# TheCacophonyProject/classifier-pipeline

Hardware: AMD Instinct MI355X
Metric: CPTV frames/s end-to-end (track+classify) at 160x120 (higher is better)
Workload: dtype u16/i32 track stage (f32 normalise, f64 gates); f32 crop/tile; f32 CNN (stride-1 3x3 convs of stages 2-4 (+ the stride-2 one): two fp16 planes per operand rounded to nearest (11 + 11 significand bits), power-of-two range scaling, 3 fp16 MFMAs per K step, device-side rerun in the exact split if an ac

## Files before the change

### classifier-pipeline_amd/csrc/cpx_api.cpp

```cpp
#include <hip/hip_runtime.h>

#include <algorithm>
#include <cmath>
#include <cstdio>
#include <cstdlib>
#include <cstring>
#include <new>
#include <string>
#include <vector>

#include "cpx_internal.h"
#include "cpx_schedule_core.h"

static_assert(sizeof(cpx_component) == 32, "cpx_component layout is part of the ABI");
static_assert(sizeof(cpx_frame_info) == 80, "cpx_frame_info layout is part of the ABI");
static_assert(sizeof(cpx_frame_meta) == 24, "cpx_frame_meta layout is part of the ABI");
static_assert(sizeof(cpx_config) == 48, "cpx_config layout is part of the ABI");
static_assert(sizeof(cpx_region_ref) == 24 && sizeof(cpx_track_limits) == 32 && sizeof(cpx_crop_req) == 32,
              "classification request layouts are part of the ABI");
static_assert(sizeof(cpx_filter_params) == 72 && sizeof(cpx_track_summary) == 120,
              "end-of-clip layouts are part of the ABI");
static_assert(sizeof(cpx_region) == 56, "cpx_region layout is part of the ABI");
static_assert(sizeof(cpx_track_record) == 32, "cpx_track_record layout is part of the ABI");
static_assert(sizeof(cpx_track_params) == 120, "cpx_track_params layout is part of the ABI");
// ... 79 lines not shown
    return CPX_ERR_HIP;
  }
  h->wtab_len = 65536;
  h->wtab_host.resize(h->wtab_len);
  std::vector<double>& wt = h->wtab_host;
  double w = 0.0;
  for (int k = 0; k < h->wtab_len; ++k) {
    wt[k] = w;
    w = w + cfg->weight_add;
  }
  if (cfg->denoise) {
    if (!cpx::nlm_supported(W, H)) {
      cpx_destroy(h);
      return CPX_ERR_UNSUPPORTED;
    }
    const int fixed_point_mult = (int)(2147483647LL / (21 * 21 * 255));
    std::vector<int> lut(64, 0);
    for (int a2 = 0; a2 < 64; ++a2) {
      const double wv = std::exp(-((double)a2 * (64.0 / 49.0)) / 9.0);
      const double wr = std::nearbyint((double)fixed_point_mult * wv);
      lut[a2] = (wr < 0.001 * fixed_point_mult) ? 0 : (int)wr;
    }
    if (lut[63] != 0 || h->nlm_lut_dev.grow(h, 64 * sizeof(int), "NLM weight table allocation") ||
        hipMemcpy(h->nlm_lut_dev.p, lut.data(), 64 * sizeof(int), hipMemcpyHostToDevice) != hipSuccess) {
      cpx_destroy(h);
      return CPX_ERR_HIP;
    }
  }
  std::vector<uint32_t> thr(h->wtab_len);
  for (int k = 0; k < h->wtab_len; ++k) {
    const double wk = wt[k], m = std::nearbyint(wk);
    const bool exact = (wk == m), near = !exact && std::fabs(wk - m) < 1e-6;
    double hi = near ? m + 1.0 : std::floor(wk) + 1.0;
    if (!(hi >= 0.0)) hi = 0.0;
    if (hi > 536870912.0) hi = 536870912.0;
    thr[k] = 2u * (uint32_t)hi - (near ? 1u : 0u);
  }
  if (h->wthr_dev.grow(h, thr.size() * sizeof(uint32_t), "threshold table allocation") ||
      hipMemcpy(h->wthr_dev.p, thr.data(), thr.size() * sizeof(uint32_t), hipMemcpyHostToDevice) != hipSuccess) {
    cpx_destroy(h);
    return CPX_ERR_HIP;
  }
  if (h->wtab_dev.grow(h, wt.size() * sizeof(double), "weight table allocation") ||
      hipMemcpy(h->wtab_dev.p, wt.data(), wt.size() * sizeof(double), hipMemcpyHostToDevice) != hipSuccess ||
      cpx::frame_kernel_attr_setup() != 0) {
    cpx_destroy(h);
    return CPX_ERR_HIP;
  }
  if (const char* env = std::getenv("CPX_TRACK_PACKED_STATE")) h->packed_state_ok = std::atoi(env) != 0;
  if (const char* env = std::getenv("CPX_CNN_FUSE_CONV1")) h->fuse_conv1 = std::atoi(env) != 0;
  if (const char* env = std::getenv("CPX_TRACK_PER_STEP")) h->track_per_step = std::atoi(env) != 0;
  if (const char* env = std::getenv("CPX_CNN_FUSE_SHORTCUT")) h->fuse_shortcut = std::atoi(env) != 0;
  if (const char* env = std::getenv("CPX_CNN_SHORTCUT_FP16")) h->shortcut_fp16 = std::atoi(env) != 0;
  if (const char* env = std::getenv("CPX_CNN_BLOCK_FUSION")) h->block_fusion = std::min(std::max(std::atoi(env), 0), 2);
  if (const char* env = std::getenv("CPX_CNN_MATH")) {
    if (!std::strcmp(env, "f32")) h->cnn_math = CPX_CNN_MATH_F32;
    else if (!std::strcmp(env, "bf16x3")) h->cnn_math = CPX_CNN_MATH_BF16X3;
    else if (!std::strcmp(env, "bf16x2")) h->cnn_math = CPX_CNN_MATH_BF16X2;
    else if (!std::strcmp(env, "fp16x2")) h->cnn_math = CPX_CNN_MATH_FP16X2;
  }
  *out = h;
  return CPX_OK;
}

static void release_buffers(cpx_handle* h, bool all) {
  for (DeviceBuffer* b : {&h->ws, &h->ws_assoc, &h->bf3_scratch, &h->cnn_arena, &h->graph_arena, &h->ir_scratch}) b->release();
  if (!all) return;
  for (DeviceBuffer* b : {&h->sched, &h->wtab_dev, &h->wthr_dev, &h->nlm_lut_dev, &h->cnn_ovf, &h->ir_bitmap}) b->release();
}

void cpx_destroy(cpx_handle* h) {
  if (!h) return;
  hipSetDevice(h->device);
  if (h->stream) hipStreamSynchronize(h->stream);
  for (cpx_cnn* c : h->cnns) cnn_free(c);
  h->cnns.clear();
  for (cpx_mog2* m : h->mog2s) mog2_free(m);
  h->mog2s.clear();
  for (cpx_graph* g : h->graphs) graph_free(g);
  h->graphs.clear();
  release_buffers(h, true);
  for (auto& e : h->conv_events) {
    hipEventDestroy(e.e0);
    hipEventDestroy(e.e1);
  }
  if (h->stream2) {
    hipStreamSynchronize(h->stream2);
    hipStreamDestroy(h->stream2);
  }
  if (h->ev_median) hipEventDestroy(h->ev_median);
  if (h->ev0) hipEventDestroy(h->ev0);
  if (h->ev1) hipEventDestroy(h->ev1);
  if (h->stream) hipStreamDestroy(h->stream);
  delete h;
}

const char* cpx_last_error(const cpx_handle* h) { return h ? h->err.c_str() : "null handle"; }

void* cpx_stream(cpx_handle* h) { return h ? (void*)h->stream : nullptr; }

static int join_medians(cpx_handle* h) {
  if (h->medians_pending) {
    h->medians_pending = false;
    CPX_HIP(h, hipStreamWaitEvent(h->stream, h->ev_median, 0));
  }
  return CPX_OK;
// ... 711 lines not shown
```

### classifier-pipeline_amd/csrc/cpx_api_cnn.cpp

```cpp
#include <hip/hip_runtime.h>

#include <algorithm>
#include <cmath>
#include <cstdio>
#include <cstdlib>
#include <new>
#include <utility>
#include <vector>

#include "cpx_internal.h"

static_assert(sizeof(cpx_wrresnet_block) == 56 && sizeof(cpx_wrresnet_params) == 1560,
              "cpx_wrresnet_params layout is part of the ABI");

struct cpx_cnn {
  cpx_handle* h = nullptr;
  cpx_wrresnet_params p{};
  std::vector<std::pair<const float*, void*>> split;
  float act_scale[3][CPX_WRRESNET_MAX_BLOCKS][2];
  float res_bound[3] = {0.0f, 0.0f, 0.0f};
  float sc_xscale[3] = {0.0f, 0.0f, 0.0f};
  void* sc_img[3] = {nullptr, nullptr, nullptr};
  double sc_wmax[3] = {-1.0, -1.0, -1.0};
  cpx_cnn() {
// ... 102 lines not shown
  Float32,
  Split,
  Fp16Pair,
  RerunOnly,
};

static int conv_run(cpx_handle* h, const cpx_conv_desc* d, const void* split_weights, const conv_fuse* fuse = nullptr,
                    const conv_half* hf = nullptr) {
  if (!h) return CPX_ERR_INVALID;
  if (!d || !d->in_dev || !d->out_dev || !d->weights_dev) return fail(h, CPX_ERR_INVALID, "cpx_conv2d: null argument");
  if (d->N < 1 || d->H < 1 || d->W < 1 || d->groups < 1 || d->Cin % d->groups || d->Cout % d->groups ||
      d->ksize < 1 || d->stride < 1 || (d->in_scale_dev == nullptr) != (d->in_shift_dev == nullptr))
    return fail(h, CPX_ERR_INVALID, "cpx_conv2d: bad descriptor");
  CPX_ENTER(h);
  if (!d->pad_same && (d->H < d->ksize || d->W < d->ksize)) return fail(h, CPX_ERR_INVALID, "cpx_conv2d: input smaller than kernel");
  cpx::ConvArgs a = conv_describe(*d, fuse);
  const bool split = split_math(h) && cpx::conv_bf3_supported(a);
  if (fuse && (!split || a.out_scale || a.residual))
    return fail(h, CPX_ERR_INVALID, "conv_run: shortcut fusion needs the split-operand kernel, no output scale, no residual");
  if (split) a.planes = h->cnn_math == CPX_CNN_MATH_BF16X2 ? 2 : 3;
  const conv_half bare;
  const conv_half& k = hf ? *hf : bare;
  const bool fp16 = split && h->cnn_math == CPX_CNN_MATH_FP16X2;
  const bool aliased = a.out == a.residual || a.out == a.in;
  const bool half = fp16 && cpx::conv_bf3_two_planes(a) && !aliased;
  const bool planes_out = fp16 && k.out_planes;
  const ConvRoute route = k.rerun_only ? ConvRoute::RerunOnly
                          : !split ? ConvRoute::Float32
                          : (half || planes_out) ? ConvRoute::Fp16Pair
                                                 : ConvRoute::Split;
  ConvTimer timer(h, h->conv_timing && route != ConvRoute::RerunOnly);
  if (!timer.ok()) return fail(h, CPX_ERR_HIP, "cpx_conv2d: event creation failed");
  int* word = nullptr;
  if (route == ConvRoute::Fp16Pair || route == ConvRoute::RerunOnly) {
    if (int rc = ensure_ovf_word(h)) return rc;
    if (!k.keep_flag) CPX_HIP(h, hipMemsetAsync(h->cnn_ovf.p, 0, sizeof(int), h->stream));
    word = h->cnn_ovf.as<int>() + k.word;
  }
  if (split && !split_weights) {
    if (int rc = h->bf3_scratch.grow(h, cpx::conv_bf3_weight_bytes(a), "cpx_conv2d: weight scratch allocation failed"))
      return rc;
    cpx::launch_split_weights(a, h->bf3_scratch.p, h->stream);
    split_weights = h->bf3_scratch.p;
  }
  int rc = 0;
  if (route == ConvRoute::Fp16Pair) {
    cpx::ConvArgs first = a;
    if (half) {
      first.planes = 2;
      first.half = 1;
      first.act_scale = k.act_scale;
      first.act_unscale = 1.0f / first.act_scale;
      first.in_planes = k.in_planes;
    }
    first.ovf = word;
    if (planes_out) {
      first.out_planes = 1;
      first.out_act_scale = k.out_act_scale;
    }
    rc = cpx::launch_conv_bf3(first, split_weights, h->stream);
  }
  a.guard = word;
  if (split) {
    if (rc == 0) rc = cpx::launch_conv_bf3(a, split_weights, h->stream);
    if (rc == -3) {
      if (fuse) return fail(h, CPX_ERR_UNSUPPORTED, "conv_run: batch too large for the fused-shortcut kernel (split the call)");
      rc = cpx::launch_conv(a, h->stream);
    }
  } else {
    rc = cpx::launch_conv(a, h->stream);
  }
  if (int trc = timer.commit((a.Cin / a.groups) * 10000 + (a.Cout / a.groups) * 10 + a.stride + (a.ksize == 1 ? 5 : 0),
                             2.0 * a.N * a.Ho * a.Wo * a.Cout * (double)(a.Cin / a.groups) * a.ksize * a.ksize))
    return trc;
  if (rc == -2) return fail(h, CPX_ERR_UNSUPPORTED, "cpx_conv2d: no kernel for this (channels per group, stride, kernel size)");
  if (rc != 0) return fail(h, CPX_ERR_HIP, "cpx_conv2d: kernel configuration failed");
  CPX_HIP(h, hipGetLastError());
  return CPX_OK;
}

static bool conv_can_fuse(const cpx_handle* h, int f, int groups) {
  return split_math(h) && cpx::conv_bf3_supported(conv_shape(0, 0, 0, f, f, groups, 3, 1, 1));
}

enum class BlockForm {
  OneLaunch,
  PlanesPair,
  Separate,
};
enum class Shortcut {
  Identity,
  FusedIntoSecond,
  OwnLaunch,
};
enum class Conv1 {
  NotHere,
  InFront,
  InsideBlock,
};
enum class Fusion { None, Block, BlockAndConv1 };

struct BlockPlan {
  int k, st, d;
  int stride, H, W, Ho, Wo, c_in, f;
  int word;
  BlockForm form;
// ... 537 lines not shown
```

### classifier-pipeline_amd/csrc/cpx_cnn_bf3.hip

```cpp
#include <hip/hip_runtime.h>

#include <algorithm>
#include <cstdlib>
#include <type_traits>

#include "cpx_cnn_dev.h"
#include "cpx_conv_layout_core.h"
#include "cpx_kernels.h"

namespace cpx {

namespace {

#define BF3_ENTRY_GUARD(H_)                          \
  if (H_) {                                          \
    if (*a.ovf != 0) return;                         \
  } else if (a.guard != nullptr && *a.guard == 0) {  \
    return;                                          \
  }

constexpr int KC = 16;

struct TileDiv {
  unsigned long long m_nsplit, m_tx, m_ty;
  int nsplit, tiles_x, tiles_y;
  int _pad;
  int total;
};
static_assert(sizeof(TileDiv) == 48 && offsetof(TileDiv, total) == 40, "the argument layout the kernels were tuned with");
#define BF3_TILE_LOOP_BEGIN for (int bid0 = blockIdx.x;;) {
#define BF3_TILE_LOOP_END        \
  if (!PERSIST) break;           \
  bid0 += gridDim.x;             \
  if (bid0 >= td.total) break;   \
  __syncthreads();               \
  }

template <int NTN, int S, int NB, int TW, int CT, bool C8, int PL = 3, bool H = false, bool PERSIST = false>
__global__ __launch_bounds__(CT) __attribute__((amdgpu_waves_per_eu(S > 1 ? CT / 256 : (CT >= 1024 ? 4 : CT / 128), S > 1 ? CT / 256 : (CT >= 1024 ? 4 : CT / 128)))) void conv_bf3_kernel(ConvArgs a, const uint4* __restrict__ wimg, TileDiv td) {
  constexpr int KS = 3;
  constexpr int WSETS = CT / 256;
  constexpr int NTM = NB / WSETS;
  static_assert(NTM * WSETS == NB, "bands must divide among the wave sets");
  constexpr int TB = 128 / TW;
  constexpr int WR = 32 / TW;
  constexpr int TH = TB * NB;
  constexpr int PH = (TH - 1) * S + KS, PW = (TW - 1) * S + KS;
  constexpr int NPX = PH * PW;
  constexpr int COGW = 32 * NTN;
  constexpr int KH = C8 ? 1 : 2;
  constexpr int QPP = C8 ? 2 : 4;
  constexpr int NSTEP = C8 ? 5 : 9;
  extern __shared__ __attribute__((aligned(16))) uint4 lds4[];
  static_assert(PL == 3 || (PL == 2 && !C8), "two planes: not for the tap-paired 8-channel form");
  static_assert(!H || PL == 2, "fp16 planes come in twos");
  BF3_ENTRY_GUARD(H)
  uint4* s_patch = lds4;
  uint4* s_w = lds4 + PL * KH * NPX;

  const int tid = threadIdx.x, lane = tid & 63, wave = (tid >> 6) & 3, wset = tid >> 8;
// ... 1421 lines not shown
#pragma unroll
          for (int pt = 0; pt < 2; ++pt) acc[ct][pt] = __builtin_amdgcn_mfma_f32_16x16x4f32(ws[ct], xs[pt], acc[ct][pt], 0, 0, 0);
      }
    }
    {
      float* out_n = b.out + (size_t)n_cur * a.H * a.W * C;
#pragma unroll
      for (int ct = 0; ct < 2; ++ct) {
#pragma unroll
        for (int pt = 0; pt < 2; ++pt) {
          f32x4 v = acc[ct][pt] * os_b[ct];
          v += ob_b[ct];
          v.x = relu_bits(v.x); v.y = relu_bits(v.y); v.z = relu_bits(v.z); v.w = relu_bits(v.w);
          if (ovalid[pt]) *reinterpret_cast<f32x4*>(at_off(out_n, (opix[pt] + 16u * ct) << 2)) = v;
        }
      }
    }
    if (!more) break;
    cbuf ^= 1;
    if (!C8) __syncthreads();
  }
  if ((hmax & 0xFFFFu) >= 0x7C00u || (hmax >> 16) >= 0x7C00u) atomicOr(a.ovf, 1);
}

using Bf3Kernel = void (*)(ConvArgs, const uint4*, TileDiv);
constexpr long long RERUN_GRID = 1024;
static int launch_bf3_tiles(Bf3Kernel kernel, Bf3Kernel rerun, bool (&ready)[2][64], const ConvArgs& a, const uint4* wimg, int tiles_x,
                            int tiles_y, int cols, unsigned threads, size_t lds, hipStream_t s) {
  if (!cpx_dyn_lds_ready(reinterpret_cast<const void*>(kernel), ready[0], 160 * 1024 - 1024)) return -1;
  TileDiv td{};
  if (const int rc = fill_tiles(td, tiles_x, tiles_y, a.N, (a.Cout / a.groups) / cols, TILES_PER_LAUNCH)) return rc;
  if (rerun != nullptr && a.guard != nullptr) {
    if (!cpx_dyn_lds_ready(reinterpret_cast<const void*>(rerun), ready[1], 160 * 1024 - 1024)) return -1;
    hipLaunchKernelGGL(rerun, dim3((unsigned)std::min<long long>(td.total, RERUN_GRID), a.groups), dim3(threads), lds, s, a, wimg, td);
    return 0;
  }
  hipLaunchKernelGGL(kernel, dim3((unsigned)td.total, a.groups), dim3(threads), lds, s, a, wimg, td);
  return 0;
}
template <int PL, bool H = false, bool SC = false>
int launch_bf3flat_t(const ConvArgs& a, const uint4* wimg, hipStream_t s) {
  constexpr int NTN = 2, NPXC = 256, CT = 256;
  constexpr int BAND = CT / 2;
  const size_t lds = std::max(((size_t)2 * PL * NPXC + (size_t)18 * PL * 32 * NTN) * 16, (size_t)(CT / 64) * 32 * 32 * sizeof(float));
  static bool lds_ready[2][64];
  Bf3Kernel rerun = nullptr;
  if constexpr (PL == 3 && !H) rerun = conv_bf3flat_kernel<NTN, NPXC, PL, false, true, CT>;
  return launch_bf3_tiles(conv_bf3flat_kernel<NTN, NPXC, PL, H, false, CT, SC>, rerun, lds_ready, a, wimg, (a.Ho * a.Wo + BAND - 1) / BAND, 1,
                          32 * NTN, CT, lds, s);
}
static bool flat_pays(const ConvArgs& a, int TW, int TH, int npx_cap, int band = 128) {
  if (a.stride != 1 || a.ksize != 3 || a.pad_top != 1 || a.pad_left != 1 || a.H != a.Ho || a.W != a.Wo) return false;
  const int M = a.Ho * a.Wo;
  const int rows = (band - 1 + a.Wo - 1) / a.Wo + 1;
  if ((rows + 2) * (a.W + 2) > npx_cap) return false;
  const double rect = (double)M / ((double)((a.Wo + TW - 1) / TW) * TW * ((a.Ho + TH - 1) / TH) * TH);
  const double flat = (double)M / ((double)((M + band - 1) / band) * band);
  return flat > rect + 0.08;
}

__global__ __launch_bounds__(256) void split_weights8_kernel(const float* __restrict__ w, uint4* __restrict__ out, int groups,
                                                             int cout_g) {
  const size_t total = (size_t)groups * 5 * 2 * cout_g;
  for (size_t idx = (size_t)blockIdx.x * blockDim.x + threadIdx.x; idx < total; idx += (size_t)gridDim.x * blockDim.x) {
    size_t r = idx;
    const int col = (int)(r % cout_g);
    r /= cout_g;
    const int h = (int)(r & 1);
    r >>= 1;
    const int st = (int)(r % 5);
    const int g = (int)(r / 5);
    const int tap = 2 * st + h;
    float v[8];
#pragma unroll
    for (int j = 0; j < 8; ++j) v[j] = tap < 9 ? w[(((size_t)g * 9 + tap) * 8 + j) * cout_g + col] : 0.0f;
    uint4 p0, p1, p2;
    split8<false>(v, 1.0f, 3, p0, p1, p2);
    const size_t base = (size_t)g * 30 * cout_g;
    out[base + ((size_t)(0 * 5 + st) * 2 + h) * cout_g + col] = p0;
    out[base + ((size_t)(1 * 5 + st) * 2 + h) * cout_g + col] = p1;
    out[base + ((size_t)(2 * 5 + st) * 2 + h) * cout_g + col] = p2;
  }
}

__global__ __launch_bounds__(256) void weight_scales_kernel(const float* __restrict__ w, float* __restrict__ wscale,
                                                            float* __restrict__ wunscale, int groups, int rows, int cout_g) {
  const int idx = blockIdx.x * blockDim.x + threadIdx.x;
  if (idx >= groups * cout_g) return;
  const int g = idx / cout_g, col = idx - g * cout_g;
  float m = 0.0f;
  for (int r = 0; r < rows; ++r) m = fmaxf(m, fabsf(w[((size_t)g * rows + r) * cout_g + col]));
  int e = 0;
  if (m > 0.0f && m < 3.0e38f) (void)frexpf(m, &e);
  else e = 4;
  const int kw = min(max(4 - e, -100), 100);
  wscale[idx] = ldexpf(1.0f, kw);
  wunscale[idx] = ldexpf(1.0f, -kw);
}

__global__ __launch_bounds__(256) void split_weights8h_kernel(const float* __restrict__ w, uint4* __restrict__ out, int groups,
                                                              const float* __restrict__ wscale) {
  const size_t total = (size_t)groups * 3 * 4 * 32;
  for (size_t idx = (size_t)blockIdx.x * blockDim.x + threadIdx.x; idx < total; idx += (size_t)gridDim.x * blockDim.x) {
    const int col = (int)(idx & 31), qq = (int)((idx >> 5) & 3), t = (int)((idx >> 7) % 3), g = (int)(idx / 384);
    const int tap = 4 * t + qq;
    const float ws = wscale[g * 32 + col];
    float v[8];
#pragma unroll
// ... 147 lines not shown
                       a.weights, image(im.planes3), sh.groups, sh.cout_g);
    hipLaunchKernelGGL(split_weights8h_kernel, dim3((unsigned)((sh.groups * 384 + 255) / 256)), dim3(256), 0, s, a.weights,
                       image(im.half), sh.groups, ws);
    return;
  }
  const unsigned grid = (unsigned)(((size_t)sh.groups * (sh.cin_g / 8) * 9 * sh.cout_g + 255) / 256);
  const auto build = [&](int chunk, size_t off, int planes, const float* wscale) {
    if (off == WeightImages::absent) return;
    if (chunk == KW)
      hipLaunchKernelGGL(split_weights32_kernel, dim3(grid), dim3(256), 0, s, a.weights, image(off), sh.groups, sh.cin_g, sh.cout_g, planes, wscale);
    else
      hipLaunchKernelGGL(split_weights_kernel, dim3(grid), dim3(256), 0, s, a.weights, image(off), sh.groups, sh.cin_g, sh.cout_g, planes, wscale);
  };
  build(im.chunk, im.planes3, 3, nullptr);
  build(im.chunk, im.planes2, 2, nullptr);
  build(im.chunk, im.half, 2, ws);
  build(KW, im.rw_half, 2, ws);
}
int launch_conv_bf3(const ConvArgs& a_in, const void* wimg, hipStream_t s) {
  ConvArgs a = a_in;
  const WeightImages im = images_of(a);
  const ConvClass cls = im.cls;
  if (cls == ConvClass::Unsupported) return -2;
  if (cls == ConvClass::Rw3 && !a.half) return launch_conv(a, s);
  if (a.half) {
    if (a.planes != 2 || !conv_bf3_two_planes(a) || a.ovf == nullptr) return -2;
    if (a.in_planes && !conv_bf3_can_load_planes(a)) return -2;
    a.w_scale = conv_bf3_weight_scales(a, wimg);
    a.w_unscale = a.w_scale + a.Cout;
  }
  if ((long long)a.H * a.W >= (1 << 24) || (long long)a.Ho * a.Wo >= (1 << 24) || a.Cin >= (1 << 24) || a.Cout >= (1 << 24)) return -3;
  if (a.in_planes && !a.half) return -2;
  if (a.out_planes && (a.ovf == nullptr || !conv_bf3_can_store_planes(a) || a.residual != nullptr)) return -2;
  const uint4* w = reinterpret_cast<const uint4*>(wimg);
  if (cls == ConvClass::C8) return launch_bf3_t<1, 1, NB_S2, TW_S2, CT_S2, true>(a, w, s);
  if (cls == ConvClass::Rw3) {
    const int rc = launch_conv_rw(a, w + im.half / 16, s);
    return rc == -2 ? launch_conv(a, s) : rc;
  }
  if (cls == ConvClass::Stride2Rw && a.planes == 2 && a.half && !a.out_planes && !a.in_planes) {
    const int rc = launch_conv_rw(a, w + im.rw_half / 16, s);
    if (rc != -2) return rc;
  }
  if (a.stride == 2)
    return with_math(a, im, w, [&](auto pl, auto h, const uint4* wi) {
      return launch_bf3_t<2, 2, 2, 16, 512, false, decltype(pl)::value, decltype(h)::value>(a, wi, s);
    });
  if (cls == ConvClass::Wide) {
    if (a.sc_in && ((a.sc_cin / a.groups) & 3)) return -2;
    return launch_bf3w(a, im, w, s);
  }
  if (cls == ConvClass::Plain) return launch_bf3_t<1, 1, NB_S2, TW_S2, CT_S2>(a, w, s);
  if (flat_pays(a, 32, 4 * NB_S4, 256)) {
    if (a.planes == 2 && a.half && a.sc_in && a.sc_planes && conv_shortcut_planes_layer(a, a.sc_cin / a.groups) && !a.residual &&
        a.sc_stride >= 1 && a.sc_xscale > 0.0f && (a.sc_H - 1) / a.sc_stride + 1 == a.Ho && (a.sc_W - 1) / a.sc_stride + 1 == a.Wo &&
        (long long)a.sc_H * a.sc_W * a.sc_cin < (1ll << 31))
      return launch_bf3flat_t<2, true, true>(a, w + im.half / 16, s);
    return with_math(a, im, w, [&](auto pl, auto h, const uint4* wi) {
      return launch_bf3flat_t<decltype(pl)::value, decltype(h)::value>(a, wi, s);
    });
  }
  return with_math(a, im, w, [&](auto pl, auto h, const uint4* wi) {
    return launch_bf3_t<NTN_S4, 1, NB_S4, 32, CT_S4, false, decltype(pl)::value, decltype(h)::value>(a, wi, s);
  });
}

bool conv_block32_supported(const ConvArgs& a, const ConvArgs& b) {
  const auto plain = [](const ConvArgs& c) {
    return c.ksize == 3 && c.stride == 1 && c.Cout / c.groups == 32 && c.relu && c.pad_top == 1 && c.pad_left == 1 && !c.out_planes &&
           !c.in_planes;
  };
  if (!(plain(a) && plain(b) && a.in_scale && a.in_shift && !a.residual && !a.sc_in && !b.in_scale && !b.out_scale &&
        a.Cout == b.Cin && b.Cin == b.Cout && a.groups == b.groups && a.H == b.H && a.W == b.W && a.N == b.N && a.ovf != nullptr))
    return false;
  if (a.Cin / a.groups == 8)
    return b.residual == nullptr && b.sc_in == a.in && b.sc_w != nullptr && b.sc_cin == a.Cin && b.sc_stride == 1 && b.sc_H == a.H &&
           b.sc_W == a.W;
  return a.Cin == a.Cout && b.residual == a.in && b.sc_in == nullptr;
}
int launch_conv_block32(const ConvArgs& a_in, const ConvArgs& b_in, const void* wimg_a, const void* wimg_b, hipStream_t s) {
  ConvArgs a = a_in, b = b_in;
  if (!conv_block32_supported(a, b)) return -2;
  if ((long long)a.H * a.W >= (1 << 24)) return -3;
  const WeightImages ia = images_of(a), ib = images_of(b);
  if (ia.half == WeightImages::absent || ib.half == WeightImages::absent) return -2;
  a.w_scale = conv_bf3_weight_scales(a, wimg_a);
  a.w_unscale = a.w_scale + a.Cout;
  b.w_scale = conv_bf3_weight_scales(b, wimg_b);
  b.w_unscale = b.w_scale + b.Cout;
  const uint4* wa = reinterpret_cast<const uint4*>(wimg_a) + ia.half / 16;
  const uint4* wb = reinterpret_cast<const uint4*>(wimg_b) + ib.half / 16;
  TileDiv td{};
  if (const int rc = fill_tiles(td, (a.W + W_TW - 1) / W_TW, (a.H + W_TH - 1) / W_TH, a.N, 1, TILES_PERSISTENT)) return rc;
  const bool c8 = a.Cin / a.groups == 8;
  static const bool split_roles = [] {
    const char* e = std::getenv("CPX_BLOCK32_SPLIT");
    return e == nullptr || std::atoi(e) != 0;
  }();
  if (!c8 && split_roles) return launch_conv_block32s(a, b, wa, wb, s);
  const bool c1 = c8 && a.c1_in != nullptr;
  if (c1 && !(a.groups == 2 && a.c1_w != nullptr && a.c1_b != nullptr)) return -2;
  const size_t lds = c8 ? (size_t)(B_R0 + B8_WIMG + B_WIMG) * 16 + 256 + (size_t)2 * B8_NPXP * 16 + (c1 ? (size_t)(B_C1W + 2 * B_C1C) * 4 : 0)
                        : (size_t)(B_R0 + 2 * B_WIMG) * 16 + 256;
  static bool lds_ready[64], lds_ready8[64], lds_ready1[64];
  if (c1 ? !cpx_dyn_lds_ready(reinterpret_cast<const void*>(conv_block32_kernel<true, true>), lds_ready1, 160 * 1024 - 1024)
      : c8 ? !cpx_dyn_lds_ready(reinterpret_cast<const void*>(conv_block32_kernel<true>), lds_ready8, 160 * 1024 - 1024)
// ... 12 lines not shown
```

### classifier-pipeline_amd/csrc/cpx_internal.h

```cpp
#pragma once
#include <hip/hip_runtime.h>

#include <map>
#include <string>
#include <vector>

#include "cpx.h"
#include "cpx_kernels.h"

struct cpx_cnn;
struct cpx_mog2;
struct cpx_graph;
void cnn_free(cpx_cnn* c);
void graph_free(cpx_graph* g);
void mog2_free(cpx_mog2* m);

struct DeviceBuffer {
  void* p = nullptr;
  size_t bytes = 0;
  DeviceBuffer() = default;
  DeviceBuffer(const DeviceBuffer&) = delete;
  DeviceBuffer& operator=(const DeviceBuffer&) = delete;
  int grow(cpx_handle* h, size_t need, const char* what);
  void release() {
    if (p) hipFree(p);
    p = nullptr;
    bytes = 0;
  }
  template <class T>
  T* as() const { return static_cast<T*>(p); }
};

struct cpx_handle {
  int device = 0;
  cpx_config cfg{};
  hipStream_t stream = nullptr;
  std::string err;
  DeviceBuffer ws;
  DeviceBuffer wtab_dev, wthr_dev;
  int wtab_len = 0;
  std::vector<double> wtab_host;
  DeviceBuffer nlm_lut_dev;
  DeviceBuffer sched;
  struct ConvEv { int key; double flops; hipEvent_t e0, e1; };
  std::vector<ConvEv> conv_events;
  bool conv_timing = false;
  DeviceBuffer ws_assoc;
  hipEvent_t ev0 = nullptr, ev1 = nullptr;
  int last_launches = 0;
  bool timing_valid = false;
  hipStream_t stream2 = nullptr;
  bool state_packed = false;
  bool packed_state_ok = true;
  bool fuse_conv1 = true;
  bool medians_pending = false;
  hipEvent_t ev_median = nullptr;
  bool track_per_step = false;
  std::vector<struct cpx_cnn*> cnns;
  std::vector<struct cpx_mog2*> mog2s;
  std::vector<struct cpx_graph*> graphs;
  DeviceBuffer graph_arena;
  int stream_frames = -1;
  int stream_assoc_frames = -1;
  bool stream_filt_state = false;
  int last_B = 0;
  struct StagedBackground { std::vector<uint16_t> bg, kcnt; double average; };
  std::map<int, StagedBackground> staged_bg;
  int cnn_math = CPX_CNN_MATH_FP16X2;
  bool fuse_shortcut = true;
  bool shortcut_fp16 = true;
  DeviceBuffer bf3_scratch;
  DeviceBuffer cnn_arena;
  DeviceBuffer cnn_ovf;
  int block_fusion = 2;
  DeviceBuffer ir_scratch;
  DeviceBuffer ir_bitmap;
};

inline int fail(cpx_handle* h, int code, const char* what, hipError_t e = hipSuccess) {
  if (h) {
    h->err = what;
    if (e != hipSuccess) {
      h->err += ": ";
      h->err += hipGetErrorString(e);
    }
  }
  return code;
}

#define CPX_HIP(h, call)                                            \
  do {                                                              \
    hipError_t _e = (call);                                         \
    if (_e != hipSuccess) return fail((h), CPX_ERR_HIP, #call, _e); \
  } while (0)

#define CPX_ENTER(h)                           \
  do {                                         \
    CPX_HIP((h), hipSetDevice((h)->device));   \
    (void)hipGetLastError();                   \
  } while (0)

inline int DeviceBuffer::grow(cpx_handle* h, size_t need, const char* what) {
  if (need <= bytes) return CPX_OK;
  if (p) CPX_HIP(h, hipStreamSynchronize(h->stream));
  release();
  const hipError_t e = hipMalloc(&p, need);
  if (e != hipSuccess) {
    p = nullptr;
    (void)hipGetLastError();
    return fail(h, CPX_ERR_NOMEM, what, e);
  }
  bytes = need;
  return CPX_OK;
}

inline size_t align_up(size_t v, size_t a) { return (v + a - 1) / a * a; }
```

### classifier-pipeline_amd/csrc/cpx_kernels.h

```cpp
#pragma once
#include <hip/hip_runtime.h>
#include <stddef.h>
#include <stdint.h>

#include "cpx.h"

#ifndef CPX_TRACK_THREADS
#define CPX_TRACK_THREADS 768
#endif
#ifndef CPX_TRACK_CHUNKS
#define CPX_TRACK_CHUNKS 7
#endif
#ifndef CPX_TRACK_LDS_COMPONENTS
#define CPX_TRACK_LDS_COMPONENTS 256
#endif
#ifndef CPX_TRACK_MIN_WAVES_PER_SIMD
#define CPX_TRACK_MIN_WAVES_PER_SIMD 6
#endif

namespace cpx {

typedef cpx_component Component;
typedef cpx_frame_info FrameInfo;

// ... 113 lines not shown
  int W, H, crop_x, crop_y, crop_w, crop_h;
  int frame_size, square_width;
  int limits_flags;
  const uint16_t* frames;
  const float* filtered;
  const FrameInfo* info;
  const cpx_region_ref* refs;
  const int* track_offsets;
  cpx_track_limits* limits;
  const cpx_crop_req* reqs;
  float* out;
};
struct AggregateArgs {
  int n_samples, n_tracks, n_labels, fp_index, square_width;
  const float* probs;
  const int* sample_track;
  const cpx_crop_req* reqs;
  float* scores;
  int* best;
};
void launch_aggregate(const AggregateArgs& a, hipStream_t s);
void launch_limits(const ClassifyArgs& a, int n_tracks, hipStream_t s);
int launch_crop(const ClassifyArgs& a, int n_reqs, hipStream_t s);

struct ConvArgs {
  int N, H, W, Cin, Cout, groups, ksize, stride, relu;
  int Ho, Wo, pad_top, pad_left;
  const float* in;
  float* out;
  const float* weights;
  const float* in_scale;
  const float* in_shift;
  const float* out_scale;
  const float* out_shift;
  const float* residual;
  const float* sc_in;
  const float* sc_w;
  const float* sc_bias;
  int sc_H, sc_W, sc_cin, sc_stride;
  const void* sc_planes;
  float sc_xscale;
  const float* c1_in;
  const float* c1_w;
  const float* c1_b;
  int planes;
  int half;
  float act_scale, act_unscale;
  const float* w_scale;
  const float* w_unscale;
  int* ovf;
  const int* guard;
  int out_planes, in_planes;
  float out_act_scale;
};
struct HeadArgs {
  int N, HW, C, L;
  int n_hidden, activation;
  int hidden_sizes[CPX_HEAD_MAX_HIDDEN];
  const float* in;
  const float* bn_scale;
  const float* bn_shift;
  const float* hidden_w[CPX_HEAD_MAX_HIDDEN];
  const float* hidden_b[CPX_HEAD_MAX_HIDDEN];
  const float* dense_w;
  const float* dense_b;
  float* logits;
  float* probs;
};
int launch_conv(const ConvArgs& a, hipStream_t s);
bool conv_bf3_supported(const ConvArgs& a);
size_t conv_bf3_weight_bytes(const ConvArgs& a);
bool conv_bf3_two_planes(const ConvArgs& a);
bool conv_bf3_can_store_planes(const ConvArgs& a);
bool conv_bf3_can_load_planes(const ConvArgs& a);
void launch_split_weights(const ConvArgs& a, void* wimg, hipStream_t s);
int launch_conv_bf3(const ConvArgs& a, const void* wimg, hipStream_t s);
bool conv_block32_supported(const ConvArgs& a, const ConvArgs& b);
int launch_conv_block32(const ConvArgs& a, const ConvArgs& b, const void* wimg_a, const void* wimg_b, hipStream_t s);
int launch_conv_block32s(const ConvArgs& a, const ConvArgs& b, const void* wa, const void* wb, hipStream_t s);
int conv_rw_kind(const ConvArgs& a);
bool conv_rw_layer(const ConvArgs& a);
int launch_conv_rw(const ConvArgs& a, const void* wimg, hipStream_t s);
bool conv_shortcut_planes_layer(const ConvArgs& second, int sc_cin_g);
size_t conv_shortcut_image_bytes(int groups, int cin_g, int cout_g);
void launch_split_shortcut(const float* sc_w, void* img, int groups, int cin_g, int cout_g, const float* w_scale, float factor,
                           hipStream_t s);
const float* conv_bf3_weight_scales(const ConvArgs& a, const void* wimg);
void launch_head(const HeadArgs& a, hipStream_t s);
void launch_count_overflow(int* ovf, int n_words, hipStream_t s);

struct CptvArgs {
  int W, H;
  const unsigned char* payload;
  const long long* frame_offsets;
  const int* bit_widths;
  const int* clip_offsets;
  uint16_t* frames_out;
};
int launch_cptv_unpack(const CptvArgs& a, int B, hipStream_t s);

struct CptvInflateArgs {
  int B;
  const unsigned char* in;
  const cpx_cptv_file* files;
  unsigned char* out;
  cpx_cptv_frame_slot* slots;
  unsigned char* header;
  cpx_cptv_file_result* results;
};
int launch_cptv_inflate(const CptvInflateArgs& a, hipStream_t s);

struct CptvGatherArgs {
  const cpx_cptv_frame_slot* slots;
  const long long* slot_offsets;
  const int* clip_offsets;
  long long* frame_offsets;
  int* bit_widths;
  cpx_cptv_frame_slot* slots_out;
};
int launch_cptv_gather(const CptvGatherArgs& a, int B, hipStream_t s);

struct ThumbArgs {
  int W, H, chain_cap;
  int max_w, max_h;
  const uint16_t* frames;
  const int32_t* labels;
  const cpx_frame_info* info;
  const cpx_region_ref* refs;
  cpx_thumb_stat* out;
};
int launch_thumb(const ThumbArgs& a, int n_refs, hipStream_t s);

struct TracklessArgs {
  int W, H, frame, background;
  const uint16_t* frames;
// ... 130 lines not shown
```

Before: 3.161 million.

## Add flat-band fp16-pair conv kernel with 128-column tiles and two-workgroup occupancy

Adds a dedicated flat-band kernel for stride-1 3x3 convolutions in fp16 two-plane mode. Each workgroup covers a 128-pixel band across 128 output columns, with double-buffered LDS patch staging and software-pipelined weight and LDS reads. Its LDS budget is sized so two workgroups fit per CU. It also handles the shortcut projection and residual-in-accumulator paths, and is enabled by default with an env switch to turn it off. The aim is better reuse and occupancy than the generic bf3flat kernel. The cost is another code path with its own overflow checking and support limits, which falls back when unsupported.

Result: faster. 3.243 million, median of 6 (+2.6%).

```diff
diff --git a/classifier-pipeline_amd/csrc/cpx_api.cpp b/classifier-pipeline_amd/csrc/cpx_api.cpp
--- a/classifier-pipeline_amd/csrc/cpx_api.cpp
+++ b/classifier-pipeline_amd/csrc/cpx_api.cpp
@@ -155,6 +155,7 @@
   if (const char* env = std::getenv("CPX_TRACK_PER_STEP")) h->track_per_step = std::atoi(env) != 0;
   if (const char* env = std::getenv("CPX_CNN_FUSE_SHORTCUT")) h->fuse_shortcut = std::atoi(env) != 0;
   if (const char* env = std::getenv("CPX_CNN_SHORTCUT_FP16")) h->shortcut_fp16 = std::atoi(env) != 0;
+  if (const char* env = std::getenv("CPX_CNN_FLAT16")) h->flat16 = std::atoi(env) != 0;
   if (const char* env = std::getenv("CPX_CNN_BLOCK_FUSION")) h->block_fusion = std::min(std::max(std::atoi(env), 0), 2);
   if (const char* env = std::getenv("CPX_CNN_MATH")) {
     if (!std::strcmp(env, "f32")) h->cnn_math = CPX_CNN_MATH_F32;
diff --git a/classifier-pipeline_amd/csrc/cpx_api_cnn.cpp b/classifier-pipeline_amd/csrc/cpx_api_cnn.cpp
--- a/classifier-pipeline_amd/csrc/cpx_api_cnn.cpp
+++ b/classifier-pipeline_amd/csrc/cpx_api_cnn.cpp
@@ -178,6 +178,7 @@
       first.act_scale = k.act_scale;
       first.act_unscale = 1.0f / first.act_scale;
       first.in_planes = k.in_planes;
+      first.flat16 = h->flat16;
     }
     first.ovf = word;
     if (planes_out) {
diff --git a/classifier-pipeline_amd/csrc/cpx_cnn_bf3.hip b/classifier-pipeline_amd/csrc/cpx_cnn_bf3.hip
--- a/classifier-pipeline_amd/csrc/cpx_cnn_bf3.hip
+++ b/classifier-pipeline_amd/csrc/cpx_cnn_bf3.hip
@@ -6,6 +6,7 @@
 
 #include "cpx_cnn_dev.h"
 #include "cpx_conv_layout_core.h"
+#include "cpx_flat_band_core.h"
 #include "cpx_kernels.h"
 
 namespace cpx {
@@ -1533,8 +1534,7 @@
 static bool flat_pays(const ConvArgs& a, int TW, int TH, int npx_cap, int band = 128) {
   if (a.stride != 1 || a.ksize != 3 || a.pad_top != 1 || a.pad_left != 1 || a.H != a.Ho || a.W != a.Wo) return false;
   const int M = a.Ho * a.Wo;
-  const int rows = (band - 1 + a.Wo - 1) / a.Wo + 1;
-  if ((rows + 2) * (a.W + 2) > npx_cap) return false;
+  if (flat_band_max_pixels(band, a.Wo) > npx_cap) return false;
   const double rect = (double)M / ((double)((a.Wo + TW - 1) / TW) * TW * ((a.Ho + TH - 1) / TH) * TH);
   const double flat = (double)M / ((double)((M + band - 1) / band) * band);
   return flat > rect + 0.08;
@@ -1788,6 +1788,10 @@
   }
   if (cls == ConvClass::Plain) return launch_bf3_t<1, 1, NB_S2, TW_S2, CT_S2>(a, w, s);
   if (flat_pays(a, 32, 4 * NB_S4, 256)) {
+    if (a.flat16 && a.planes == 2 && a.half) {
+      const int rc = launch_conv_flat16(a, w + im.half / 16, s);
+      if (rc != -2) return rc;
+    }
     if (a.planes == 2 && a.half && a.sc_in && a.sc_planes && conv_shortcut_planes_layer(a, a.sc_cin / a.groups) && !a.residual &&
         a.sc_stride >= 1 && a.sc_xscale > 0.0f && (a.sc_H - 1) / a.sc_stride + 1 == a.Ho && (a.sc_W - 1) / a.sc_stride + 1 == a.Wo &&
         (long long)a.sc_H * a.sc_W * a.sc_cin < (1ll << 31))
diff --git a/classifier-pipeline_amd/csrc/cpx_cnn_flat.hip b/classifier-pipeline_amd/csrc/cpx_cnn_flat.hip
--- /dev/null
+++ b/classifier-pipeline_amd/csrc/cpx_cnn_flat.hip
@@ -0,0 +1,306 @@
+#include <hip/hip_runtime.h>
+
+#include <algorithm>
+
+#include "cpx_cnn_dev.h"
+#include "cpx_conv_layout_core.h"
+#include "cpx_flat_band_core.h"
+#include "cpx_kernels.h"
+
+namespace cpx {
+
+namespace {
+
+constexpr int F_CT = 256, F_BAND = 128, F_COLS = 128;
+constexpr int F_NPXC = 256;
+constexpr int F_NPXP = 262;
+constexpr int F_PLANE = 2 * F_NPXP * 2;
+constexpr int F_BUF = 2 * F_PLANE;
+constexpr int F_BANDP = 130;
+constexpr int F_SCPLANE = 2 * F_BANDP * 2;
+static_assert(F_NPXP >= F_NPXC && 2 * 2 * F_SCPLANE <= F_BUF, "a patch buffer holds a band's patch, or the shortcut's operand");
+constexpr int F_BNC = 256;
+#ifndef CPX_FLAT16_PT
+#define CPX_FLAT16_PT 8
+#endif
+#ifndef CPX_FLAT16_AHEAD
+#define CPX_FLAT16_AHEAD 1
+#endif
+constexpr size_t F_LDS = (size_t)2 * F_BUF * 16 + (size_t)2 * F_BNC * sizeof(float);
+static_assert(2 * F_LDS <= 160 * 1024, "two workgroups per CU");
+
+template <bool SC, int PT>
+__global__ __launch_bounds__(F_CT) __attribute__((amdgpu_waves_per_eu(2, 2))) void conv_flat16_kernel(ConvArgs a, const uint4* __restrict__ wimg, Tiles td) {
+  constexpr int CTN = 16 / PT;
+  constexpr int NWP = 8 / PT;
+  constexpr int NP = 4 * F_NPXC / F_CT;
+  static_assert(PT * CTN == 16 && NWP * (F_COLS / (16 * CTN)) == F_CT / 64, "four waves cover 8 x 8 tiles");
+  static_assert(NP * F_CT == 8 * F_BAND, "the shortcut's operand is staged through the same registers");
+  extern __shared__ __attribute__((aligned(16))) uint4 lds4[];
+  if (*a.ovf != 0) return;
+
+  const int tid = threadIdx.x, lane = tid & 63, wave = tid >> 6;
+  const int l15 = lane & 15, lq = lane >> 4;
+  const int wp = wave % NWP, wc = wave / NWP;
+  int bid = blockIdx.x;
+  if ((gridDim.x & 7) == 0) bid = (bid & 7) * (gridDim.x >> 3) + (bid >> 3);
+  const int ti = tile_split(bid, td.m_tx, td.tiles_x);
+  const int n = bid;
+  const int g = blockIdx.y;
+  const int cin_g = a.Cin / a.groups;
+  const int M = a.Ho * a.Wo;
+  const FlatBand fb = flat_band(ti, F_BAND, a.Ho, a.Wo);
+  const float* in_n = a.in + (size_t)n * a.H * a.W * a.Cin + (size_t)g * cin_g;
+  const int nchunks = cin_g / 32;
+  const int chw = g * F_COLS + wc * (16 * CTN) + 4 * lq;
+  const int pw0 = fb.p0 + wp * (16 * PT) + l15;
+
+  const bool res_in_acc = a.residual != nullptr && a.out_scale == nullptr;
+  f32x4 acc[PT][CTN];
+  if (res_in_acc) {
+    const float* res_n = a.residual + (size_t)n * M * a.Cout;
+    f32x4 rs[CTN];
+#pragma unroll
+    for (int ct = 0; ct < CTN; ++ct) rs[ct] = *reinterpret_cast<const f32x4*>(a.w_scale + chw + ct * 16) * a.act_scale;
+#pragma unroll
+    for (int pt = 0; pt < PT; ++pt) {
+      const unsigned ro = (__umul24((unsigned)min(pw0 + pt * 16, M - 1), (unsigned)a.Cout) + (unsigned)chw) << 2;
+#pragma unroll
+      for (int ct = 0; ct < CTN; ++ct) acc[pt][ct] = *reinterpret_cast<const f32x4*>(at_off(res_n, ro + ct * 64)) * rs[ct];
+    }
+  } else {
+#pragma unroll
+    for (int pt = 0; pt < PT; ++pt)
+#pragma unroll
+      for (int ct = 0; ct < CTN; ++ct) acc[pt][ct] = f32x4{0.0f, 0.0f, 0.0f, 0.0f};
+  }
+
+  int bb[PT];
+#pragma unroll
+  for (int pt = 0; pt < PT; ++pt) bb[pt] = ((lq >> 1) * F_NPXP + flat_patch_base(fb, pw0 + pt * 16, M, a.Wo)) * 2 + (lq & 1);
+  const uint4* wg = wimg + (size_t)g * (cin_g / 16) * 36 * F_COLS;
+  const unsigned wlane = (unsigned)(((lq >> 1) * 36 + (lq & 1)) * F_COLS + wc * (16 * CTN) + l15) << 4;
+  u32x4 wf[2][CTN][2];
+  const auto load_w = [&](u32x4 (&w)[CTN][2], int cc, int tap) {
+    const u32x4* wt = reinterpret_cast<const u32x4*>(wg + (size_t)(cc * 72 + tap * 2) * F_COLS);
+#pragma unroll
+    for (int p = 0; p < 2; ++p)
+#pragma unroll
+      for (int ct = 0; ct < CTN; ++ct) w[ct][p] = *at_off(wt, wlane + (unsigned)((p * 18 * F_COLS + ct * 16) << 4));
+  };
+
+  const int my_q = tid & 3;
+  unsigned soff[NP], inside = 0;
+  int se[NP];
+#pragma unroll
+  for (int i = 0; i < NP; ++i) {
+    const int px = min((tid + i * F_CT) >> 2, fb.npx - 1);
+    int iy, ix;
+    flat_item_pixel(fb, px, iy, ix);
+    if (iy >= 0 && iy < a.H && ix >= 0 && ix < a.W) inside |= 1u << i;
+    soff[i] = (pix_off(min(max(iy, 0), a.H - 1), min(max(ix, 0), a.W - 1), a.W, a.Cin) + (unsigned)(8 * my_q)) << 2;
+    se[i] = ((my_q >> 1) * F_NPXP + px) * 2 + (my_q & 1);
+  }
+  f32x4 pre_p[NP][2];
+  f32x4* s_bn = reinterpret_cast<f32x4*>(lds4 + 2 * F_BUF);
+  if (a.in_scale && tid < cin_g / 4) {
+    s_bn[tid] = *reinterpret_cast<const f32x4*>(a.in_scale + g * cin_g + 4 * tid) * a.act_scale;
+    s_bn[F_BNC / 4 + tid] = *reinterpret_cast<const f32x4*>(a.in_shift + g * cin_g + 4 * tid) * a.act_scale;
+  }
+  const auto load_patch = [&](int cc) {
+    const int cn = cc * 32;
+#pragma unroll
+    for (int i = 0; i < NP; ++i) {
+      pre_p[i][0] = *reinterpret_cast<const f32x4*>(at_off(in_n + cn, soff[i]));
+      pre_p[i][1] = *reinterpret_cast<const f32x4*>(at_off(in_n + cn, soff[i] + 16));
+    }
+  };
+  const auto split_entry = [](const float (&v)[8], float& vmax, u32x4& hi, u32x4& lo) {
+#pragma unroll
+    for (int j = 0; j < 8; j += 2) vmax = fmaxf(fmaxf(fabsf(v[j]), fabsf(v[j + 1])), vmax);
+    unsigned q0[4], q1[4];
+#pragma unroll
+    for (int j = 0; j < 4; ++j) split2<true>(v[2 * j], v[2 * j + 1], q0[j], q1[j]);
+    hi = u32x4{q0[0], q0[1], q0[2], q0[3]};
+    lo = u32x4{q1[0], q1[1], q1[2], q1[3]};
+  };
+
+  load_patch(0);
+  __syncthreads();
+  for (int cc = 0; cc < nchunks; ++cc) {
+    load_w(wf[0], cc, 0);
+    u32x4* buf = reinterpret_cast<u32x4*>(lds4) + (cc & 1) * F_BUF;
+    {
+      float vmax = 0.0f;
+      f32x4 psc[2], psh[2];
+#pragma unroll
+      for (int k = 0; k < 2; ++k) {
+        psc[k] = s_bn[cc * 8 + my_q * 2 + k];
+        psh[k] = s_bn[F_BNC / 4 + cc * 8 + my_q * 2 + k];
+      }
+#pragma unroll
+      for (int i = 0; i < NP; ++i) {
+        const bool in = (inside >> i) & 1;
+        float v[8];
+#pragma unroll
+        for (int j = 0; j < 8; ++j) v[j] = pre_p[i][j >> 2][j & 3];
+        if (a.in_scale) {
+#pragma unroll
+          for (int j = 0; j < 8; ++j) v[j] = fmaxf(__fmaf_rn(v[j], psc[j >> 2][j & 3], psh[j >> 2][j & 3]), 0.0f);
+        } else {
+#pragma unroll
+          for (int j = 0; j < 8; ++j) v[j] *= a.act_scale;
+        }
+#pragma unroll
+        for (int j = 0; j < 8; ++j) v[j] = in ? v[j] : 0.0f;
+        u32x4 hi, lo;
+        split_entry(v, vmax, hi, lo);
+        buf[se[i]] = hi;
+        buf[F_PLANE + se[i]] = lo;
+      }
+      if (vmax > F16_MAX) atomicOr(a.ovf, 1);
+    }
+    __syncthreads();
+    if (cc + 1 < nchunks) {
+      load_patch(cc + 1);
+    } else if (SC) {
+      const float* sc_n = a.sc_in + (size_t)n * a.sc_H * a.sc_W * a.sc_cin + g * 64 + 8 * (tid & 7);
+#pragma unroll
+      for (int i = 0; i < NP; ++i) {
+        const int sp = min(fb.p0 + ((tid + i * F_CT) >> 3), M - 1);
+        const int sy = sp / a.Wo, sx = sp - sy * a.Wo;
+        const float* src = sc_n + ((size_t)(sy * a.sc_stride) * a.sc_W + sx * a.sc_stride) * a.sc_cin;
+        pre_p[i][0] = *reinterpret_cast<const f32x4*>(src);
+        pre_p[i][1] = *reinterpret_cast<const f32x4*>(src + 4);
+      }
+    }
+    u32x4 bv[2][2];
+    const auto read_b = [&](u32x4 (&b)[2], int tap, int pt) {
+      const int e = bb[pt] + flat_tap_offset(fb, tap / 3, tap % 3) * 2;
+#pragma unroll
+      for (int p = 0; p < 2; ++p) b[p] = buf[p * F_PLANE + e];
+    };
+    read_b(bv[0], 0, 0);
+#pragma unroll
+    for (int tap = 0; tap < 9; ++tap) {
+      if (tap + 1 < 9) load_w(wf[(tap + 1) & 1], cc, tap + 1);
+#pragma unroll
+      for (int pt = 0; pt < PT; ++pt) {
+        const int st = tap * PT + pt;
+        if (st + 1 < 9 * PT) read_b(bv[(st + 1) & 1], (st + 1) / PT, (st + 1) % PT);
+        if (CPX_FLAT16_AHEAD) __builtin_amdgcn_sched_barrier(0);
+#pragma unroll
+        for (int ct = 0; ct < CTN; ++ct) plane_products16<2, true>(bv[st & 1], wf[tap & 1][ct], acc[pt][ct]);
+      }
+    }
+  }
+
+  if constexpr (SC) {
+    const u32x4* scw = reinterpret_cast<const u32x4*>(a.sc_planes) + (size_t)g * 16 * F_COLS;
+    const unsigned sclane = (unsigned)(lq * F_COLS + wc * (16 * CTN) + l15) << 4;
+#pragma unroll
+    for (int c = 0; c < 2; ++c)
+#pragma unroll
+      for (int p = 0; p < 2; ++p)
+#pragma unroll
+        for (int ct = 0; ct < CTN; ++ct) wf[c][ct][p] = *at_off(scw, sclane + (unsigned)((((c * 2 + p) * 4) * F_COLS + ct * 16) << 4));
+    u32x4* sbuf = reinterpret_cast<u32x4*>(lds4) + (nchunks & 1) * F_BUF;
+    {
+      const int j = tid & 7, c = j >> 2, qq = j & 3;
+      float vmax = 0.0f;
+#pragma unroll
+      for (int i = 0; i < NP; ++i) {
+        float v[8];
+#pragma unroll
+        for (int k = 0; k < 8; ++k) v[k] = pre_p[i][k >> 2][k & 3] * a.sc_xscale;
+        u32x4 hi, lo;
+        split_entry(v, vmax, hi, lo);
+        const int e = ((c * 2 * 2 + (qq >> 1)) * F_BANDP + ((tid + i * F_CT) >> 3)) * 2 + (qq & 1);
+        sbuf[e] = hi;
+        sbuf[F_SCPLANE + e] = lo;
+      }
+      if (!(vmax <= F16_MAX)) atomicOr(a.ovf, 1);
+    }
+    __syncthreads();
+#pragma unroll
+    for (int c = 0; c < 2; ++c) {
+      u32x4 bv[PT][2];
+#pragma unroll
+      for (int pt = 0; pt < PT; ++pt)
+#pragma unroll
+        for (int p = 0; p < 2; ++p)
+          bv[pt][p] = sbuf[((c * 2 + p) * 2 + (lq >> 1)) * (F_BANDP * 2) + (wp * (16 * PT) + pt * 16 + l15) * 2 + (lq & 1)];
+#pragma unroll
+      for (int pt = 0; pt < PT; ++pt)
+#pragma unroll
+        for (int ct = 0; ct < CTN; ++ct) plane_products16<2, true>(bv[pt], wf[c][ct], acc[pt][ct]);
+    }
+  }
+
+  float* out_n = a.out + (size_t)n * M * a.Cout;
+  const float* res_n = (a.residual && !res_in_acc) ? a.residual + (size_t)n * M * a.Cout : nullptr;
+  f32x4 os[CTN], ob[CTN];
+#pragma unroll
+  for (int ct = 0; ct < CTN; ++ct) {
+    const int ch = chw + ct * 16;
+    const f32x4 one = {1.0f, 1.0f, 1.0f, 1.0f}, zero = {0.0f, 0.0f, 0.0f, 0.0f};
+    os[ct] = a.out_scale ? *reinterpret_cast<const f32x4*>(a.out_scale + ch) : one;
+    os[ct] *= *reinterpret_cast<const f32x4*>(a.w_unscale + ch) * a.act_unscale;
+    ob[ct] = (a.out_shift ? *reinterpret_cast<const f32x4*>(a.out_shift + ch) : zero) +
+             (a.sc_in && a.sc_bias ? *reinterpret_cast<const f32x4*>(a.sc_bias + ch) : zero);
+  }
+#pragma unroll
+  for (int pt = 0; pt < PT; ++pt) {
+    const int p = pw0 + pt * 16;
+    if (p < M) {
+      const unsigned o = (__umul24((unsigned)p, (unsigned)a.Cout) + (unsigned)chw) << 2;
+      f32x4 v[CTN];
+#pragma unroll
+      for (int ct = 0; ct < CTN; ++ct) v[ct] = acc[pt][ct] * os[ct] + ob[ct];
+      if (res_n) {
+        f32x4 rv[CTN];
+#pragma unroll
+        for (int ct = 0; ct < CTN; ++ct) rv[ct] = *reinterpret_cast<const f32x4*>(at_off(res_n, o + ct * 64));
+#pragma unroll
+        for (int ct = 0; ct < CTN; ++ct) v[ct] += rv[ct];
+      }
+#pragma unroll
+      for (int ct = 0; ct < CTN; ++ct) {
+        if (a.relu) {
+          v[ct].x = relu_bits(v[ct].x); v[ct].y = relu_bits(v[ct].y); v[ct].z = relu_bits(v[ct].z); v[ct].w = relu_bits(v[ct].w);
+        }
+        *reinterpret_cast<f32x4*>(at_off(out_n, o + ct * 64)) = v[ct];
+      }
+    }
+  }
+}
+
+template <bool SC, int PT>
+int launch_flat16_t(const ConvArgs& a, const uint4* wimg, hipStream_t s) {
+  Tiles td{};
+  if (const int rc = fill_tiles(td, flat_bands(F_BAND, a.Ho, a.Wo), 1, a.N, TILES_PER_LAUNCH)) return rc;
+  static bool lds_ready[64];
+  if (!cpx_dyn_lds_ready(reinterpret_cast<const void*>(conv_flat16_kernel<SC, PT>), lds_ready, 160 * 1024 - 1024)) return -1;
+  hipLaunchKernelGGL((conv_flat16_kernel<SC, PT>), dim3((unsigned)td.total, (unsigned)a.groups), dim3(F_CT), F_LDS, s, a, wimg, td);
+  return 0;
+}
+
+}
+
+int launch_conv_flat16(const ConvArgs& a, const void* wimg, hipStream_t s) {
+  if (!a.flat16 || !a.half || a.planes != 2 || a.ovf == nullptr || a.guard != nullptr || a.in_planes || a.out_planes) return -2;
+  if (a.ksize != 3 || a.stride != 1 || a.pad_top != 1 || a.pad_left != 1 || a.H != a.Ho || a.W != a.Wo || a.groups < 1) return -2;
+  if (a.Cout != F_COLS * a.groups || a.Cin % (32 * a.groups) || a.Cin < 32 * a.groups || a.Cin > F_BNC * a.groups) return -2;
+  if (flat_band_max_pixels(F_BAND, a.Wo) > F_NPXC) return -2;
+  if ((long long)a.H * a.W >= (1 << 24) || a.Cin >= (1 << 24) || (long long)a.H * a.W * std::max(a.Cin, a.Cout) >= (1ll << 30)) return -2;
+  const uint4* wi = reinterpret_cast<const uint4*>(wimg);
+  if (a.sc_in) {
+    if (!a.sc_planes || !conv_shortcut_planes_layer(a, a.sc_cin / a.groups) || a.residual || a.sc_stride < 1 || !(a.sc_xscale > 0.0f) ||
+        (a.sc_H - 1) / a.sc_stride + 1 != a.Ho || (a.sc_W - 1) / a.sc_stride + 1 != a.Wo || (long long)a.sc_H * a.sc_W * a.sc_cin >= (1ll << 31))
+      return -2;
+    return launch_flat16_t<true, CPX_FLAT16_PT>(a, wi, s);
+  }
+  return launch_flat16_t<false, CPX_FLAT16_PT>(a, wi, s);
+}
+
+}
diff --git a/classifier-pipeline_amd/csrc/cpx_flat_band_core.h b/classifier-pipeline_amd/csrc/cpx_flat_band_core.h
--- /dev/null
+++ b/classifier-pipeline_amd/csrc/cpx_flat_band_core.h
@@ -0,0 +1,49 @@
+#pragma once
+
+namespace cpx {
+
+#if defined(__HIPCC__)
+#define CPX_FLAT_HD __host__ __device__ __forceinline__
+#else
+#define CPX_FLAT_HD inline
+#endif
+
+struct FlatBand {
+  int p0;
+  int y_first, y_last;
+  int PW, PH;
+  int npx;
+};
+CPX_FLAT_HD FlatBand flat_band(int ti, int band, int Ho, int Wo) {
+  const int M = Ho * Wo;
+  FlatBand b;
+  b.p0 = ti * band;
+  const int plast = b.p0 + band - 1 < M - 1 ? b.p0 + band - 1 : M - 1;
+  b.y_first = b.p0 / Wo;
+  b.y_last = plast / Wo;
+  b.PW = Wo + 2;
+  b.PH = b.y_last - b.y_first + 3;
+  b.npx = b.PH * b.PW;
+  return b;
+}
+CPX_FLAT_HD int flat_bands(int band, int Ho, int Wo) { return (Ho * Wo + band - 1) / band; }
+CPX_FLAT_HD int flat_band_max_pixels(int band, int Wo) {
+  const int rows = (band - 1 + Wo - 1) / Wo + 1;
+  return (rows + 2) * (Wo + 2);
+}
+CPX_FLAT_HD void flat_item_pixel(const FlatBand& b, int px, int& iy, int& ix) {
+  const int py = px / b.PW;
+  iy = b.y_first - 1 + py;
+  ix = px - py * b.PW - 1;
+}
+CPX_FLAT_HD int flat_patch_base(const FlatBand& b, int p, int M, int Wo) {
+  const int pc = p < M - 1 ? p : M - 1;
+  const int y = pc / Wo, x = pc - y * Wo;
+  return (y - b.y_first) * b.PW + x;
+}
+CPX_FLAT_HD int flat_tap_offset(const FlatBand& b, int ky, int kx) { return ky * b.PW + kx; }
+CPX_FLAT_HD int flat_patch_offset(const FlatBand& b, int p, int M, int Wo, int ky, int kx) {
+  return flat_patch_base(b, p, M, Wo) + flat_tap_offset(b, ky, kx);
+}
+
+}
diff --git a/classifier-pipeline_amd/csrc/cpx_internal.h b/classifier-pipeline_amd/csrc/cpx_internal.h
--- a/classifier-pipeline_amd/csrc/cpx_internal.h
+++ b/classifier-pipeline_amd/csrc/cpx_internal.h
@@ -69,6 +69,7 @@
   int cnn_math = CPX_CNN_MATH_FP16X2;
   bool fuse_shortcut = true;
   bool shortcut_fp16 = true;
+  bool flat16 = true;
   DeviceBuffer bf3_scratch;
   DeviceBuffer cnn_arena;
   DeviceBuffer cnn_ovf;
diff --git a/classifier-pipeline_amd/csrc/cpx_kernels.h b/classifier-pipeline_amd/csrc/cpx_kernels.h
--- a/classifier-pipeline_amd/csrc/cpx_kernels.h
+++ b/classifier-pipeline_amd/csrc/cpx_kernels.h
@@ -189,7 +189,9 @@
   const int* guard;
   int out_planes, in_planes;
   float out_act_scale;
-};
+  int flat16;
+};
+static_assert(sizeof(ConvArgs) == 264, "the argument layout the convolution kernels were tuned with");
 struct HeadArgs {
   int N, HW, C, L;
   int n_hidden, activation;
@@ -218,6 +220,7 @@
 int conv_rw_kind(const ConvArgs& a);
 bool conv_rw_layer(const ConvArgs& a);
 int launch_conv_rw(const ConvArgs& a, const void* wimg, hipStream_t s);
+int launch_conv_flat16(const ConvArgs& a, const void* wimg, hipStream_t s);
 bool conv_shortcut_planes_layer(const ConvArgs& second, int sc_cin_g);
 size_t conv_shortcut_image_bytes(int groups, int cin_g, int cout_g);
 void launch_split_shortcut(const float* sc_w, void* img, int groups, int cin_g, int cout_g, const float* w_scale, float factor,
```
